# ForJadeForest/DistillCLIP

Measured on AMD Instinct MI355X. Metric: image-text pairs/sec (distill step), higher is better.
Workload: dtype bf16; 1 GPU; l_clip.yaml dual distill: ViT-B/32 CLIP teacher -> weight-shared ViT(6x768,24h,R2) + text(4x768,12h,R2) students, 224px/77tok, losses out_l1+out_cos+0.1*cos_diff, fwd+loss+bwd+AdamW; global_batch=512, batch_per_gpu=512, parallelism=dp1, gradient_exchange=none, negatives=local (reference training_step semantics), optimizer_in_step=True, teacher_residual=fp16, saved_gelu_derivative=u8 fixed point, clock_probe=True

## Files before the change

distillclip_amd/csrc/encoder.cpp:

```cpp
#include <math.h>
#include <stdlib.h>
#include <string.h>
#include <new>
#include <vector>
#include "common.h"

namespace {

#define CK(expr)                      \
    do {                              \
        int _rc = (expr);             \
        if (_rc != DCLIP_OK) return _rc; \
    } while (0)

inline size_t up256(size_t x) { return (x + 255) & ~(size_t)255; }

struct Bump {
    char* base; size_t off;
    explicit Bump(void* b) : base((char*)b), off(0) {}
    template <class T> T* take(size_t n) {
        T* p = base ? (T*)(base + off) : nullptr;
        off += up256(n * sizeof(T));
        return p;
    }
// ... 605 lines not shown
    return DCLIP_OK;
}

extern "C" int dclip_encoder_backward(const dclip_encoder* e, const void* input, const void* patches, int64_t B, const void* const* params,
                                      void* const* grads, const void* wcache, void* workspace, size_t ws_bytes, dclip_encoder_run* run,
                                      const float* d_last_representation, const float* const* d_rep, const float* d_emb,
                                      const dclip_attn_maps* maps, dclip_bucket_cb on_bucket, void* cb_user, void* st) {
    DCLIP_REQUIRE(e && (input || patches) && params && grads && wcache && workspace && run && d_last_representation, "dclip_encoder_backward: null argument");
    const Plan& p = e->p;
    const bf16_t* ext_patches = (const bf16_t*)patches;
    DCLIP_REQUIRE(!ext_patches || p.image, "dclip_encoder_backward: patches: image towers only");
    DCLIP_REQUIRE(p.train, "dclip_encoder_backward: the frozen teacher tower (kind 0) has no backward");
    ExecMaps<const float> gm;
    CK(exec_maps<const float>(p, maps, maps ? maps->d_score : nullptr, maps ? maps->d_prob : nullptr, run, "dclip_encoder_backward", gm));
    if (p.mixing && gm.prob_bits) {
        const size_t need = dclip_attn_maps_bwd_workspace_bytes(B, p.H, p.N);
        DCLIP_REQUIRE(maps->scratch && maps->scratch_bytes >= need,
                      "dclip_encoder_backward: probability-map gradients of a head-mixing tower need %zu bytes of maps scratch", need);
    }
    Work w;
    layout(p, B, true, workspace, w);
    DCLIP_REQUIRE(ws_bytes >= w.bytes, "dclip_encoder_backward: workspace too small");
    const bf16_t* W = (const bf16_t*)wcache;
    const int64_t N = p.N, D = p.D, F = p.F, E = p.E, M = B * N;
    const int nex = p.L * p.R;
    const bool pruned = (run->flags & RUN_PRUNED) != 0;
    DCLIP_REQUIRE(!pruned || !(d_rep && d_rep[nex - 1]),
                  "dclip_encoder_backward: a gradient for the hidden state of block execution %d, which the forward ran on the class / EOT "
                  "rows only (request that hidden state in the forward, or set DCLIP_PRUNE_LAST=0)", nex - 1);
    DCLIP_REQUIRE(!pruned || !(gm.score[nex - 1] || gm.prob[nex - 1]),
                  "dclip_encoder_backward: a map gradient for block execution %d, which the forward ran on the class / EOT rows only", nex - 1);
    auto GR = [&](int i) -> float* { return i < 0 ? nullptr : (float*)grads[i]; };
    hipStream_t hs = (hipStream_t)st;

    if (run->flags & RUN_SEEDS_CLEAR) run->flags &= ~RUN_SEEDS_CLEAR;
    else CK(clear_backward_seeds(p, w, M, B, pruned, st));
    CK(dclip_cast_bf16(d_last_representation, w.dout, B * E, st));
    if (p.student) {
        if (GR(p.head.head_w)) CK(dclip_gemm_tn_acc(w.dout, E, w.hf, D, GR(p.head.head_w), D, B, E, D, 1, w.tn_ws, w.tn_ws_bytes, st));
        if (GR(p.head.head_b)) CK(dclip_colsum_acc(w.dout, E, GR(p.head.head_b), B, E, st));
    } else if (GR(p.head.head_w)) {
        CK(dclip_gemm_tn_acc(w.hf, D, w.dout, E, GR(p.head.head_w), E, B, D, E, 1, w.tn_ws, w.tn_ws_bytes, st));
    }
    CK(gemm(w.dout, E, W + p.w_head_t, E, w.dh, D, B, D, E, nullptr, 0, nullptr, nullptr, nullptr, 0, DCLIP_OUT_BF16, 0, nullptr, st));
    const int R = p.R;
    bf16_t* gb_last = w.gb_f2 + (int64_t)(R - 1) * M * D;
    CK(dclip_layernorm_bwd(w.dh, D, 0, (const float*)(pruned ? w.compact.xout : w.X[nex]), D, pruned ? nullptr : w.pick, PF(params, p.head.norm_w), w.meanf,
                           w.rstdf, pruned ? w.Gc : w.G, D, gb_last, D, GR(p.head.norm_w), GR(p.head.norm_b), GR(bexec(p, (nex - 1) / p.R, 0).f2b), B, D, st));
    if (on_bucket) on_bucket(cb_user, 0);

    for (int ei = nex - 1; ei >= 0; --ei) {
        const int l = ei / p.R, r = ei % p.R;
        const auto& bw = p.bw[l];
        const ExecSave& s = w.ex[ei];
        const BX bx = bexec(p, l, r);
        const float *wl = nullptr, *ww = nullptr;
        float *gl = nullptr, *gw = nullptr;
        if (p.mixing) { wl = PF(params, bx.cl); ww = PF(params, bx.cw); gl = GR(bx.cl); gw = GR(bx.cw); }
        bf16_t* gb_f2 = w.gb_f2 + (int64_t)r * M * D;
        bf16_t* gb_pr = w.gb_pr + (int64_t)r * M * D;
        bf16_t* dbig = w.dbig + (int64_t)r * M * F;
        bf16_t* dqkv = w.dqkv + (int64_t)r * M * 3 * D;
        const int64_t MR = (int64_t)R * M;
        const ExecSave& s0 = w.ex[ei - r];
        const bool compact = pruned && ei == nex - 1;
        const RowSet rs = compact ? w.compact : full_rows(w, ei, M);
        const int64_t Mx = rs.rows;
        const int64_t MRw = pruned && l == p.L - 1 ? (int64_t)(R - 1) * M + B : MR;
        if (d_rep && d_rep[ei]) CK(dclip_axpy_f32(w.G, d_rep[ei], gb_f2, M * D, GR(bx.f2b), D, st));
        CK(dclip_gemm_nt(gb_f2, D, W + bw.fc2_t, D, dbig, F, Mx, F, D, 1.f, nullptr, DCLIP_ACT_MULAUX, rs.z, nullptr, nullptr, 0, DCLIP_OUT_BF16, 0, nullptr,
                         GR(bx.f1b), st));
        if (r == 0 && GR(bx.f2w)) CK(dclip_gemm_tn_acc(w.gb_f2, D, s0.u, F, GR(bx.f2w), F, MRw, D, F, wsplits(MRw, D, F), w.tn_ws, w.tn_ws_bytes, st));
        if (r == 0 && GR(bx.f1w)) CK(dclip_gemm_tn_acc(w.dbig, F, s0.h2, D, GR(bx.f1w), D, MRw, F, D, wsplits(MRw, F, D), w.tn_ws, w.tn_ws_bytes, st));
        CK(gemm(dbig, F, W + bw.fc1_t, F, w.dh, D, Mx, D, F, nullptr, 0, nullptr, nullptr, nullptr, 0, DCLIP_OUT_BF16, 0, nullptr, st));
        CK(dclip_layernorm_bwd(w.dh, D, 0, (const float*)rs.x_mid, D, nullptr, PF(params, bx.n2w), rs.mean2, rs.rstd2, compact ? w.Gc : w.G, D, gb_pr, D,
                               GR(bx.n2w), GR(bx.n2b), GR(bx.prb), Mx, D, st));
        if (r == 0 && GR(bx.prw)) CK(dclip_gemm_tn_acc(w.gb_pr, D, s0.ctx, D, GR(bx.prw), D, MRw, D, D, wsplits(MRw, D, D), w.tn_ws, w.tn_ws_bytes, st));
        bf16_t* dctx = w.dh;
        if (!compact) {
            CK(gemm(gb_pr, D, W + bw.proj_t, D, dctx, D, M, D, D, nullptr, 0, nullptr, nullptr, nullptr, 0, DCLIP_OUT_BF16, 0, nullptr, st));
        } else {
            bf16_t* dctx_c = dqkv;
            CK(gemm(gb_pr, D, W + bw.proj_t, D, dctx_c, D, B, D, D, nullptr, 0, nullptr, nullptr, nullptr, 0, DCLIP_OUT_BF16, 0, nullptr, st));
            CK(dclip_rows_expand(dctx_c, dctx, w.pick, B, N, D * 2, st));
            CK(dclip_rows_expand(w.Gc, w.G, w.pick, B, N, D * 4, st));
        }
        const MapGrad mg{gm.score[ei], gm.prob[ei], maps ? maps->scratch : nullptr, maps ? maps->scratch_bytes : 0};
        CK(attn_backward(w.path, p, s, w, wl, ww, gl, gw, dctx, dqkv, B, mg.d_score || mg.d_prob ? &mg : nullptr,
                         compact && (run->flags & RUN_PRUNED_ATTN) ? w.pick : nullptr, st));
        if (r == 0 && GR(bx.qkvw)) CK(dclip_gemm_tn_acc(w.dqkv, 3 * D, s0.h1, D, GR(bx.qkvw), D, MR, 3 * D, D, wsplits(MR, 3 * D, D), w.tn_ws, w.tn_ws_bytes, st));
        if (r == 0 && params[bx.qkvb] && GR(bx.qkvb)) CK(dclip_colsum_acc(w.dqkv, 3 * D, GR(bx.qkvb), MR, 3 * D, st));
        CK(gemm(dqkv, 3 * D, W + bw.qkv_t, 3 * D, w.dh, D, M, D, 3 * D, nullptr, 0, nullptr, nullptr, nullptr, 0, DCLIP_OUT_BF16, 0, nullptr, st));
        bf16_t* gb_next = ei > 0 ? w.gb_f2 + (int64_t)((ei - 1) % R) * M * D : w.Gb;
        CK(dclip_layernorm_bwd(w.dh, D, 0, (const float*)w.X[ei], D, nullptr, PF(params, bx.n1w), s.mean1, s.rstd1, w.G, D, gb_next, D, GR(bx.n1w), GR(bx.n1b),
                               ei > 0 ? GR(bexec(p, (ei - 1) / p.R, 0).f2b) : nullptr, M, D, st));
        if (r == 0 && on_bucket) on_bucket(cb_user, 1 + (p.L - 1 - l));
    }

    const Plan::EmbP& em = p.emb;
    const bool pre_ln = em.ln_w >= 0;
    if (d_emb && !pre_ln) CK(dclip_axpy_f32(w.G, d_emb, w.Gb, M * D, nullptr, D, st));
    if (hipMemsetAsync(w.tok_sum, 0, (size_t)N * D * 4, hs) != hipSuccess) { dclip_set_error("dclip_encoder_backward: memset failed"); return DCLIP_ELAUNCH; }
    const float* Ge = w.G;
    if (pre_ln) {
        if (hipMemsetAsync(w.G0, 0, (size_t)M * D * 4, hs) != hipSuccess) { dclip_set_error("dclip_encoder_backward: memset failed"); return DCLIP_ELAUNCH; }
        CK(dclip_layernorm_bwd(w.G, D, 1, (const float*)w.x0, D, nullptr, PF(params, em.ln_w), w.mean0, w.rstd0, w.G0, D, w.Gb, D, GR(em.ln_w), GR(em.ln_b),
                               nullptr, M, D, st));
        if (d_emb) CK(dclip_axpy_f32(w.G0, d_emb, w.Gb, M * D, nullptr, D, st));
        Ge = w.G0;
    }
    if (em.w >= 0) {
        const int64_t K = p.K;
        const bf16_t* rows = ext_patches ? ext_patches : w.patches;
        if (GR(em.w)) CK(dclip_gemm_tn_acc(w.Gb, D, rows, K, GR(em.w), K, M, D, K, wsplits(M, D, K), w.tn_ws, w.tn_ws_bytes, st));
        if (GR(em.bias) || GR(em.cls) || GR(em.pos)) {
            CK(dclip_batch_sum_acc(Ge, w.tok_sum, B, N, D, st));
            CK(dclip_token_table_bwd(w.tok_sum, GR(em.pos), GR(em.cls), GR(em.bias), N, D, p.image ? 1 : 0, st));
        }
        if (GR(em.table)) {
            CK(gemm(w.Gb, D, W + p.w_embed_t, D, w.demb, K, M, K, D, nullptr, 0, nullptr, nullptr, nullptr, 0, DCLIP_OUT_F32, 0, nullptr, st));
            CK(dclip_embed_scatter_add((const int64_t*)input, w.demb, 1, GR(em.table), M, K, p.c.vocab, st));
        }
    } else {
// ... 22 lines not shown
```

distillclip_amd/csrc/gemm.hip:

```cpp

#include "gemm_common.h"
#include <atomic>

using namespace dgemm;

namespace {

constexpr int TILE_BYTES = (BM / 16) * (BK / 32) * SUB;
constexpr int CLD = BN + 4;
constexpr int NT_LDS = (4 * TILE_BYTES > BM * CLD * 4) ? 4 * TILE_BYTES : BM * CLD * 4;


__device__ __forceinline__ void stage_operand(const bf16_t* __restrict__ G, int64_t ld, int row0, int rows_max,
                                              int k0, char* lds_tile, int wave, int lane) {
    const int L = lane * 16;
    const int X = swz(L);
    const int r = X >> 6, c = (X >> 4) & 3;
#pragma unroll
    for (int s = 0; s < 4; ++s) {
        const int sub = wave * 4 + s;
        const int rb = sub >> 1, kb = sub & 1;
        int row = row0 + rb * 16 + r;
        row = row < rows_max ? row : rows_max - 1;
        const bf16_t* src = G + (int64_t)row * ld + (k0 + kb * 32 + c * 8);
// ... 614 lines not shown
    float* cs = (float*)smem;
#pragma unroll
    for (int i = 0; i < 4; ++i)
#pragma unroll
        for (int j = 0; j < 4; ++j)
#pragma unroll
            for (int r = 0; r < 4; ++r)
                cs[(wp * 64 + i * 16 + (lane >> 4) * 4 + r) * TCLD + wq * 64 + j * 16 + (lane & 15)] = acc[i][j][r];
    __syncthreads();
#pragma unroll 4
    for (int it = 0; it < 64; ++it) {
        const int rl = wave * 32 + (it >> 1), cl = (it & 1) * 64 + lane;
        const int row = p0 + rl, col = q0 + cl;
        if (row < p.P && col < p.Q) unsafeAtomicAdd(p.out + (int64_t)row * p.ldo + col, cs[rl * TCLD + cl]);
    }
}

__device__ __forceinline__ void tn_half_sources(const bf16_t* __restrict__ G, int64_t ld, int m0, int c0, int wave, int lane,
                                                const char* (&src)[2]) {
#pragma unroll
    for (int s = 0; s < 2; ++s) {
        const int piece = wave * 2 + s;
        const int r = piece * 4 + (lane >> 4);
        const int lc = (lane & 15) ^ tn_key(r);
        src[s] = (const char*)(G + (int64_t)(m0 + r) * ld + c0 + lc * 8);
    }
}
__device__ __forceinline__ void stage_half_tn(const char* const (&src)[2], int64_t chunk_off, char* buf, int wave) {
#pragma unroll
    for (int s = 0; s < 2; ++s)
        __builtin_amdgcn_global_load_lds((gbl_void*)(src[s] + chunk_off), (lds_void*)(buf + (wave * 2 + s) * 1024), 16, 0, 0);
}

__global__ __launch_bounds__(512) void gemm_tn256_kernel(GemmTN p) {
    extern __shared__ __attribute__((aligned(16))) char smem[];
    const int tid = threadIdx.x, lane = tid & 63;
    const int wave = __builtin_amdgcn_readfirstlane(tid >> 6);
    const int wr = wave >> 2, wc = wave & 3;

    const int tiles = p.tiles_p * p.tiles_q;
    const int t = xcd_remap(blockIdx.x, tiles * p.splits);
    const int split = t / tiles, tile = t - split * tiles;
    const int tq = tile % p.tiles_q, tp = tile / p.tiles_q;
    const int p0 = tp * 256, q0 = tq * 256;
    const int m_begin = split * p.chunk;
    const int m_end = min(p.M, m_begin + p.chunk);
    if (m_begin >= m_end) return;
    const int nk = (m_end - m_begin) / TC;
    const int nload = 4 * nk;

    f32x4 acc[8][4];
#pragma unroll
    for (int i = 0; i < 8; ++i)
#pragma unroll
        for (int j = 0; j < 4; ++j) acc[i][j] = f32x4{0.f, 0.f, 0.f, 0.f};

    const char* srcs[4][2];
    tn_half_sources(p.B, p.ldb, m_begin, q0, wave, lane, srcs[0]);
    tn_half_sources(p.B, p.ldb, m_begin, q0 + 128, wave, lane, srcs[1]);
    tn_half_sources(p.A, p.lda, m_begin, p0, wave, lane, srcs[2]);
    tn_half_sources(p.A, p.lda, m_begin, p0 + 128, wave, lane, srcs[3]);
    const int64_t step_b = (int64_t)TC * p.ldb * 2, step_a = (int64_t)TC * p.lda * 2;
    auto issue = [&](int l) {
        const int kt = l >> 2, w = l & 3;
        char* buf = smem + ((kt & 1) * 4 + w) * HT;
        if (w == 0) stage_half_tn(srcs[0], kt * step_b, buf, wave);
        else if (w == 1) stage_half_tn(srcs[1], kt * step_b, buf, wave);
        else if (w == 2) stage_half_tn(srcs[2], kt * step_a, buf, wave);
        else stage_half_tn(srcs[3], kt * step_a, buf, wave);
    };
    auto stamp = [&](int k) {
        if (p.stamps && tid == 0) {
            if (k == 3) WAIT_VMCNT(0);
            p.stamps[6 * (int64_t)blockIdx.x + k] = __builtin_readcyclecounter();
            if (k == 0) p.stamps[6 * (int64_t)blockIdx.x + 4] = __builtin_amdgcn_s_memrealtime();
            if (k == 3) p.stamps[6 * (int64_t)blockIdx.x + 5] = __builtin_amdgcn_s_memrealtime();
        }
    };
    stamp(0);
    const int npro = nload < 6 ? nload : 6;
#pragma unroll
    for (int l = 0; l < 6; ++l)
        if (l < npro) issue(l);
    if (nload > 4) WAIT_VMCNT(4); else WAIT_VMCNT(0);
    __builtin_amdgcn_s_barrier();
    stamp(1);
    if (wr == 1) __builtin_amdgcn_s_barrier();

    const int a_off = (2 + wr) * HT;
    const int b_off = (wc >> 1) * HT;
    const int bcol = (wc & 1) * 64;
    bf16x8 af[4][2], b0[2][2], b1[2][2];

    for (int kt = 0; kt < nk; ++kt) {
        const char* base = smem + (kt & 1) * 4 * HT;
        const char* at = base + a_off;
        const char* bt = base + b_off;
        const int k4 = kt * 4;
#pragma unroll
        for (int j = 0; j < 2; ++j) {
            const unsigned a0 = tr_frag_base(bt, bcol + j * 16, lane), a1 = tr_frag_base(bt, bcol + (2 + j) * 16, lane);
            b0[j][0] = tr_frag_asm<0>(a0); b0[j][1] = tr_frag_asm<32 * 256>(a0);
            b1[j][0] = tr_frag_asm<0>(a1); b1[j][1] = tr_frag_asm<32 * 256>(a1);
        }
        __builtin_amdgcn_sched_barrier(0);
#pragma unroll
        for (int i = 0; i < 4; ++i) {
            const unsigned a0 = tr_frag_base(at, i * 16, lane);
            af[i][0] = tr_frag_asm<0>(a0); af[i][1] = tr_frag_asm<32 * 256>(a0);
// ... 29 lines not shown
        __builtin_amdgcn_sched_barrier(0);
        __builtin_amdgcn_s_barrier();
        __builtin_amdgcn_s_setprio(1);
#pragma unroll
        for (int kb = 0; kb < 2; ++kb)
#pragma unroll
            for (int i = 0; i < 4; ++i) {
#pragma unroll
                for (int j = 0; j < 2; ++j)
                    acc[4 + i][j] = __builtin_amdgcn_mfma_f32_16x16x32_bf16(af[i][kb], b0[j][kb], acc[4 + i][j], 0, 0, 0);
#pragma unroll
                for (int j = 0; j < 2; ++j)
                    acc[4 + i][2 + j] = __builtin_amdgcn_mfma_f32_16x16x32_bf16(af[i][kb], b1[j][kb], acc[4 + i][2 + j], 0, 0, 0);
            }
        __builtin_amdgcn_s_setprio(0);
        __builtin_amdgcn_s_barrier();
    }
    if (wr == 0) __builtin_amdgcn_s_barrier();
    stamp(2);

    float* cs = (float*)smem;
    constexpr int CL = 256 + 4;
#pragma unroll
    for (int q = 0; q < 4; ++q) {
        __syncthreads();
#pragma unroll
        for (int i = 0; i < 2; ++i)
#pragma unroll
            for (int j = 0; j < 4; ++j)
#pragma unroll
                for (int r = 0; r < 4; ++r)
                    cs[(wr * 32 + i * 16 + (lane >> 4) * 4 + r) * CL + wc * 64 + j * 16 + (lane & 15)] = acc[q * 2 + i][j][r];
        __syncthreads();
        if (p.partial) {
            float* dst = p.partial + ((int64_t)split * tiles + tile) * 65536;
#pragma unroll 4
            for (int it = 0; it < 8; ++it) {
                const int sl = (tid >> 6) + it * 8;
                const int rt = (sl >> 5) * 128 + q * 32 + (sl & 31);
                *(float4*)(dst + rt * 256 + (tid & 63) * 4) = *(const float4*)&cs[sl * CL + (tid & 63) * 4];
            }
        } else {
#pragma unroll 4
            for (int it = 0; it < 32; ++it) {
                const int sl = (tid >> 8) + it * 2;
                const int row = p0 + (sl >> 5) * 128 + q * 32 + (sl & 31);
                const int col = q0 + (tid & 255);
                unsafeAtomicAdd(p.out + (int64_t)row * p.ldo + col, cs[sl * CL + (tid & 255)]);
            }
        }
    }
    stamp(3);
}

__global__ __launch_bounds__(256) void tn256_reduce_kernel(const float* __restrict__ partial, int splits, int tiles, int tiles_q,
                                                           float* __restrict__ out, int64_t ldo) {
    const int idx = blockIdx.x * 256 + threadIdx.x;
    const int tile = idx >> 14, rt = (idx >> 6) & 255, c4 = idx & 63;
    if (tile >= tiles) return;
    const float* src = partial + (int64_t)tile * 65536 + rt * 256 + c4 * 4;
    float4 a = *(const float4*)src;
    for (int s = 1; s < splits; ++s) {
        const float4 v = *(const float4*)(src + (int64_t)s * tiles * 65536);
        a.x += v.x; a.y += v.y; a.z += v.z; a.w += v.w;
    }
    float* o = out + (int64_t)((tile / tiles_q) * 256 + rt) * ldo + (tile % tiles_q) * 256 + c4 * 4;
    float4 cur = *(const float4*)o;
    cur.x += a.x; cur.y += a.y; cur.z += a.z; cur.w += a.w;
    *(float4*)o = cur;
}

__global__ __launch_bounds__(256) void colsum_kernel(const bf16_t* __restrict__ X, int64_t ld, float* __restrict__ db,
                                                     int M, int N, int rows_per_block) {
    const int col = blockIdx.x * 256 + threadIdx.x;
    if (col >= N) return;
    const int r0 = blockIdx.y * rows_per_block;
    const int r1 = min(M, r0 + rows_per_block);
    float s0 = 0.f, s1 = 0.f, s2 = 0.f, s3 = 0.f;
    int r = r0;
    for (; r + 3 < r1; r += 4) {
        s0 += bf2f(X[(int64_t)r * ld + col]);
        s1 += bf2f(X[(int64_t)(r + 1) * ld + col]);
        s2 += bf2f(X[(int64_t)(r + 2) * ld + col]);
        s3 += bf2f(X[(int64_t)(r + 3) * ld + col]);
    }
// ... 200 lines not shown
    chunk = ((chunk + TC - 1) / TC) * TC;
    p.chunk = chunk;
    p.splits = (int)((M + chunk - 1) / chunk);
    const int grid = p.tiles_p * p.tiles_q * p.splits;
    const bool fast = M % TC == 0 && P >= 8 && Q >= 8;
    if (fast && P % 256 == 0 && Q % 256 == 0 && (P / 256) * (Q / 256) >= 16 && M >= 4096) {
        GemmTN q = p;
        q.tiles_p = (int)(P / 256); q.tiles_q = (int)(Q / 256);
        const int tiles = q.tiles_p * q.tiles_q;
        int s = (256 + tiles / 2) / tiles;
        if (s < 1) s = 1;
        int ch = (int)((M + s - 1) / s);
        ch = ((ch + TC - 1) / TC) * TC;
        q.chunk = ch;
        q.splits = (int)((M + ch - 1) / ch);
        TraceScope tr2(DCLIP_TRACE_GEMM_TN, 2.0 * (double)M * (double)P * (double)Q, 2.0 * ((double)M * P + (double)M * Q) + 4.0 * (double)P * Q, stream, (int)M, (int)P, (int)Q, 256);
        static const int tn_partial = [] { const char* e = getenv("DCLIP_TN_PARTIAL"); return e ? atoi(e) : 1; }();
        const size_t need = (size_t)tiles * q.splits * 65536 * sizeof(float);
        const bool part = tn_partial != 0 && workspace && ws_bytes >= need && ldo % 4 == 0 && ((uintptr_t)dW % 16) == 0 && q.splits > 1;
        if (!part && q.splits > 1) g_tn_atomic_fallbacks.fetch_add(1, std::memory_order_relaxed);
        q.partial = part ? (float*)workspace : nullptr;
        hipLaunchKernelGGL(gemm_tn256_kernel, dim3(tiles * q.splits), dim3(512), 8 * HT, (hipStream_t)stream, q);
        if (part)
            hipLaunchKernelGGL(tn256_reduce_kernel, dim3((unsigned)(tiles * 64)), dim3(256), 0, (hipStream_t)stream, (const float*)workspace,
                               q.splits, tiles, q.tiles_q, dW, ldo);
        return dclip_check_launch("dclip_gemm_tn_acc");
    }
    TraceScope tr(DCLIP_TRACE_GEMM_TN, 2.0 * (double)M * (double)P * (double)Q, 2.0 * ((double)M * P + (double)M * Q) + 4.0 * (double)P * Q, stream, (int)M, (int)P, (int)Q, 128);
    if (fast) hipLaunchKernelGGL(gemm_tn_glds_kernel, dim3(grid), dim3(256), TN_LDS, (hipStream_t)stream, p);
    else hipLaunchKernelGGL(gemm_tn_kernel, dim3(grid), dim3(256), 4 * TTILE, (hipStream_t)stream, p);
    return dclip_check_launch("dclip_gemm_tn_acc");
}

extern "C" int dclip_colsum_acc(const void* X, int64_t ld, float* db, int64_t M, int64_t N, void* stream) {
    DCLIP_REQUIRE(X && db && M > 0 && N > 0, "dclip_colsum_acc: bad argument");
    const int colblocks = (int)((N + 255) / 256);
    int rows_per_block = (int)((M * colblocks + 511) / 512);
    rows_per_block = rows_per_block < 16 ? 16 : (rows_per_block > 512 ? 512 : (rows_per_block + 3) & ~3);
    dim3 grid((unsigned)((N + 255) / 256), (unsigned)((M + rows_per_block - 1) / rows_per_block));
    if (N % 8 == 0 && ld % 8 == 0 && ((uintptr_t)X & 15) == 0)
        hipLaunchKernelGGL(colsum8_kernel, grid, dim3(256), 0, (hipStream_t)stream, (const bf16_t*)X, ld, db, (int)M, (int)N,
                           rows_per_block);
    else
        hipLaunchKernelGGL(colsum_kernel, grid, dim3(256), 0, (hipStream_t)stream, (const bf16_t*)X, ld, db, (int)M, (int)N,
                           rows_per_block);
    return dclip_check_launch("dclip_colsum_acc");
}
```

distillclip_amd/ops.py:

```python
import torch

from ._lib import lib

ACT = {'none': 0, None: 0, 'quickgelu': 1, 'gelu': 2, 'dgelu': 3, 'mulaux': 4, 'gelu_save': 5, 'quickgelu_save': 6}
OUT_DTYPE = {torch.bfloat16: 0, torch.float32: 1, torch.float16: 2}
DG_LO, DG_STEP = -0.13, 1.26 / 255.0


def _p(t):
    return 0 if t is None else t.data_ptr()


def _stream():
    return torch.cuda.current_stream().cuda_stream


def _chk(*ts):
    for t in ts:
        if t is not None and not t.is_cuda:
            raise RuntimeError('distillclip_amd ops need CUDA(HIP) tensors; there is no CPU fallback')


def gemm_nt(a, b, *, bias=None, act=None, aux_in=None, aux_out=None, residual=None, out=None, out_dtype=torch.bfloat16,
            alpha=1.0, row_group=0, rowadd=None, out_rows=None, colsum=None):
    _chk(a, b, bias, aux_in, aux_out, residual, out, rowadd)
    assert a.dtype == torch.bfloat16 and b.dtype == torch.bfloat16 and a.dim() == 2 and b.dim() == 2
    assert a.stride(1) == 1 and b.stride(1) == 1
    M, K = a.shape
    N = b.shape[0]
    if out is None:
        rows = out_rows if out_rows is not None else M
        out = torch.empty((rows, N), dtype=out_dtype, device=a.device)
# ... 2 lines not shown
    if act in ('gelu_save', 'quickgelu_save') and aux_out is not None:
        assert aux_out.dtype == torch.uint8 and aux_out.stride(0) == out.stride(0)
    if act == 'mulaux':
        assert aux_in.dtype == torch.uint8 and aux_in.stride(0) == out.stride(0)
    if residual is not None:
        assert residual.dtype == (torch.float16 if out.dtype == torch.float16 else torch.float32)
    lib().dclip_gemm_nt(_p(a), a.stride(0), _p(b), b.stride(0), _p(out), out.stride(0), M, N, K, float(alpha),
                        _p(bias), ACT[act], _p(aux_in), _p(aux_out), _p(residual), ldr,
                        OUT_DTYPE[out.dtype], row_group, _p(rowadd), _p(colsum), _stream())
    return out


_TN_WS = {}


def _tn_workspace(device):
    key = (device, _stream())
    ws = _TN_WS.get(key)
    if ws is None:
        ws = _TN_WS[key] = torch.empty(lib().dclip_gemm_tn_workspace_bytes(), dtype=torch.uint8, device=device)
    return ws


def gemm_tn_acc(a, b, dw, splits=4, workspace=True):
    _chk(a, b, dw)
    assert a.dtype == torch.bfloat16 and b.dtype == torch.bfloat16 and dw.dtype == torch.float32
    M, P = a.shape
    Q = b.shape[1]
    assert b.shape[0] == M and tuple(dw.shape) == (P, Q) and dw.stride(1) == 1
    ws = _tn_workspace(a.device) if workspace else None
    lib().dclip_gemm_tn_acc(_p(a), a.stride(0), _p(b), b.stride(0), _p(dw), dw.stride(0), M, P, Q, splits, _p(ws),
                            0 if ws is None else ws.numel(), _stream())
    return dw


def colsum_acc(x, db):
    _chk(x, db)
    assert x.dtype == torch.bfloat16 and db.dtype == torch.float32
    lib().dclip_colsum_acc(_p(x), x.stride(0), _p(db), x.shape[0], x.shape[1], _stream())
    return db


def layernorm_fwd(x, gamma, beta, *, row_index=None, out_dtype=torch.bfloat16, eps=1e-5, save_stats=True):
    _chk(x, gamma, beta, row_index)
    assert x.dtype in (torch.float32, torch.float16) and x.dim() == 2 and x.stride(1) == 1
    M = row_index.numel() if row_index is not None else x.shape[0]
    D = x.shape[1]
    y = torch.empty((M, D), dtype=out_dtype, device=x.device)
    mean = torch.empty(M, dtype=torch.float32, device=x.device) if save_stats else None
    rstd = torch.empty(M, dtype=torch.float32, device=x.device) if save_stats else None
    fn = lib().dclip_layernorm_fwd_f16 if x.dtype == torch.float16 else lib().dclip_layernorm_fwd
    fn(_p(x), x.stride(0), _p(row_index), _p(gamma), _p(beta), _p(y), D, OUT_DTYPE[out_dtype], _p(mean), _p(rstd), M, D, eps, _stream())
    return y, mean, rstd


def layernorm_bwd(dy, x, gamma, mean, rstd, dx_acc, *, row_index=None, dx_bf16=None, dgamma=None, dbeta=None, colsum=None):
    _chk(dy, x, gamma, mean, rstd, dx_acc, dx_bf16, dgamma, dbeta)
    M, D = dy.shape
    lib().dclip_layernorm_bwd(_p(dy), dy.stride(0), 1 if dy.dtype == torch.float32 else 0, _p(x), x.stride(0),
                              _p(row_index), _p(gamma), _p(mean), _p(rstd), _p(dx_acc), dx_acc.stride(0), _p(dx_bf16),
                              dx_bf16.stride(0) if dx_bf16 is not None else 0, _p(dgamma), _p(dbeta), _p(colsum), M, D, _stream())


def attn_nt(a, lda, bm, ldb, B, H, N, hd, alpha=1.0, out_dtype=torch.float32):
    Np = (N + 7) // 8 * 8
    c = torch.empty((B, H, N, Np), dtype=out_dtype, device=a.device)
# ... 280 lines not shown
```

include/dclip.h:

```cpp
#ifndef DCLIP_H
#define DCLIP_H
#include <stddef.h>
#include <stdint.h>
#ifdef __cplusplus
extern "C" {
#endif

#define DCLIP_OK 0
#define DCLIP_EINVAL (-1)
#define DCLIP_ELAUNCH (-2)

int dclip_version(void);
int dclip_runtime_check(void);
const char* dclip_arch(void);
const char* dclip_last_error_string(void);

#define DCLIP_ACT_NONE 0
#define DCLIP_ACT_QUICKGELU 1
#define DCLIP_ACT_GELU 2
#define DCLIP_ACT_DGELU 3
#define DCLIP_ACT_MULAUX 4
#define DCLIP_ACT_GELU_SAVE 5
#define DCLIP_ACT_QUICKGELU_SAVE 6
#define DCLIP_OUT_BF16 0
#define DCLIP_OUT_F32 1
#define DCLIP_OUT_F16 2

int dclip_gemm_nt(const void* A, int64_t lda, const void* B, int64_t ldb, void* C, int64_t ldc,
                  int64_t M, int64_t N, int64_t K, float alpha, const float* bias, int act,
                  const void* aux_in, void* aux_out, const void* residual, int64_t ldr, int out_dtype,
                  int64_t row_group, const float* rowadd, float* colsum_acc, void* stream);

size_t dclip_gemm_tn_workspace_bytes(void);
int64_t dclip_gemm_tn_atomic_fallbacks(void);
int dclip_gemm_tn_acc(const void* A, int64_t lda, const void* B, int64_t ldb, float* dW, int64_t ldo,
                      int64_t M, int64_t P, int64_t Q, int splits, void* workspace, size_t ws_bytes, void* stream);

int dclip_colsum_acc(const void* X, int64_t ld, float* db, int64_t M, int64_t N, void* stream);

int dclip_layernorm_fwd(const float* x, int64_t ldx, const int32_t* row_index, const float* gamma, const float* beta,
                        void* y, int64_t ldy, int out_f32, float* mean, float* rstd, int64_t M, int64_t D, float eps,
                        void* stream);
int dclip_layernorm_fwd_f16(const void* x, int64_t ldx, const int32_t* row_index, const float* gamma, const float* beta,
                            void* y, int64_t ldy, int out_dtype, float* mean, float* rstd, int64_t M, int64_t D, float eps,
                            void* stream);
int dclip_layernorm_bwd(const void* dy, int64_t lddy, int dy_f32, const float* x, int64_t ldx, const int32_t* row_index,
                        const float* gamma, const float* mean, const float* rstd, float* dx_acc, int64_t lddx,
                        void* dx_bf16, int64_t lddb, float* dgamma, float* dbeta, float* colsum_acc, int64_t M, int64_t D,
                        void* stream);

int dclip_attn_nt(const void* A, int64_t lda, const void* Bm, int64_t ldb, void* C, int out_f32, int64_t B, int64_t H,
                  int64_t N, int64_t Np, int64_t hd, float alpha, void* stream);
int dclip_attn_nn(const void* A, const void* Bm, int64_t ldb, void* C, int64_t ldc, int64_t B, int64_t H, int64_t N,
                  int64_t Np, int64_t hd, float alpha, int a_blocked, void* stream);
int dclip_attn_tn(const void* A, const void* Bm, int64_t ldb, void* C, int64_t ldc, int64_t B, int64_t H, int64_t N,
                  int64_t Np, int64_t hd, float alpha, int a_blocked, void* stream);
int dclip_attn_fused_fwd(const void* qkv, int64_t ldq, void* ctx, int64_t ldc, int64_t B, int64_t H, int64_t N, int64_t hd,
                         float scale, int causal, void* stream);
int dclip_attn_stream_fwd(const void* qkv, int64_t ldq, void* ctx, int64_t ldc, int64_t B, int64_t H, int64_t N, int64_t hd,
                          float scale, void* stream);
int dclip_attn_softmax_fwd(const float* S, const float* Wl, const float* Ww, void* P, void* R, int64_t B, int64_t H,
                           int64_t N, int64_t Np, int causal, void* stream);
int dclip_attn_softmax_bwd(const void* dR, const void* P, const void* S, int scores_bf16, const float* Wl, const float* Ww,
                           void* dS, float* dWl, float* dWw, int64_t B, int64_t H, int64_t N, int64_t Np, void* stream);
int dclip_attn_mix_supported(int64_t H, int64_t N, int64_t hd);
size_t dclip_attn_mix_bwd_workspace_bytes(int64_t B, int64_t H, int64_t N);
void dclip_attn_mix_debug_stamps(void* fwd, void* bwd_a, void* bwd_b);
int dclip_attn_mix_fwd(const void* qkv, int64_t ld, const float* Wl, const float* Ww, void* R, float* stats, int64_t B, int64_t H,
                       int64_t N, int64_t Np, int64_t hd, float scale, void* stream);
// ... 167 lines not shown
```

Before: 18620 pairs/s.

## Group per-layer weight-gradient TN GEMMs into one persistent split-K launch

Batches the four weight-gradient TN GEMMs of each layer (fc2, fc1, qkv, proj) into a single grouped kernel. The kernel balances K-slabs of all problems across a fixed number of workgroups, writes partials to a workspace and reduces them in a follow-up kernel. It aims to cut launch count and load imbalance, and to raise CU utilisation over separate split-K launches with atomics. The cost is that all four GEMMs now wait until after attention backward, plus extra partial-buffer traffic. It is on by default, can be switched off with an env var, and falls back to separate calls if constraints fail.

```diff
diff --git a/distillclip_amd/csrc/encoder.cpp b/distillclip_amd/csrc/encoder.cpp
--- a/distillclip_amd/csrc/encoder.cpp
+++ b/distillclip_amd/csrc/encoder.cpp
@@ -661,6 +661,7 @@
                   "dclip_encoder_backward: a map gradient for block execution %d, which the forward ran on the class / EOT rows only", nex - 1);
     auto GR = [&](int i) -> float* { return i < 0 ? nullptr : (float*)grads[i]; };
     hipStream_t hs = (hipStream_t)st;
+    static const bool tn_grouped = [] { const char* e = getenv("DCLIP_TN_GROUPED"); return e ? atoi(e) != 0 : true; }();
 
     if (run->flags & RUN_SEEDS_CLEAR) run->flags &= ~RUN_SEEDS_CLEAR;
     else CK(clear_backward_seeds(p, w, M, B, pruned, st));
@@ -696,15 +697,16 @@
         const RowSet rs = compact ? w.compact : full_rows(w, ei, M);
         const int64_t Mx = rs.rows;
         const int64_t MRw = pruned && l == p.L - 1 ? (int64_t)(R - 1) * M + B : MR;
+        const bool wg_each = r == 0 && !tn_grouped;
         if (d_rep && d_rep[ei]) CK(dclip_axpy_f32(w.G, d_rep[ei], gb_f2, M * D, GR(bx.f2b), D, st));
         CK(dclip_gemm_nt(gb_f2, D, W + bw.fc2_t, D, dbig, F, Mx, F, D, 1.f, nullptr, DCLIP_ACT_MULAUX, rs.z, nullptr, nullptr, 0, DCLIP_OUT_BF16, 0, nullptr,
                          GR(bx.f1b), st));
-        if (r == 0 && GR(bx.f2w)) CK(dclip_gemm_tn_acc(w.gb_f2, D, s0.u, F, GR(bx.f2w), F, MRw, D, F, wsplits(MRw, D, F), w.tn_ws, w.tn_ws_bytes, st));
-        if (r == 0 && GR(bx.f1w)) CK(dclip_gemm_tn_acc(w.dbig, F, s0.h2, D, GR(bx.f1w), D, MRw, F, D, wsplits(MRw, F, D), w.tn_ws, w.tn_ws_bytes, st));
+        if (wg_each && GR(bx.f2w)) CK(dclip_gemm_tn_acc(w.gb_f2, D, s0.u, F, GR(bx.f2w), F, MRw, D, F, wsplits(MRw, D, F), w.tn_ws, w.tn_ws_bytes, st));
+        if (wg_each && GR(bx.f1w)) CK(dclip_gemm_tn_acc(w.dbig, F, s0.h2, D, GR(bx.f1w), D, MRw, F, D, wsplits(MRw, F, D), w.tn_ws, w.tn_ws_bytes, st));
         CK(gemm(dbig, F, W + bw.fc1_t, F, w.dh, D, Mx, D, F, nullptr, 0, nullptr, nullptr, nullptr, 0, DCLIP_OUT_BF16, 0, nullptr, st));
         CK(dclip_layernorm_bwd(w.dh, D, 0, (const float*)rs.x_mid, D, nullptr, PF(params, bx.n2w), rs.mean2, rs.rstd2, compact ? w.Gc : w.G, D, gb_pr, D,
                                GR(bx.n2w), GR(bx.n2b), GR(bx.prb), Mx, D, st));
-        if (r == 0 && GR(bx.prw)) CK(dclip_gemm_tn_acc(w.gb_pr, D, s0.ctx, D, GR(bx.prw), D, MRw, D, D, wsplits(MRw, D, D), w.tn_ws, w.tn_ws_bytes, st));
+        if (wg_each && GR(bx.prw)) CK(dclip_gemm_tn_acc(w.gb_pr, D, s0.ctx, D, GR(bx.prw), D, MRw, D, D, wsplits(MRw, D, D), w.tn_ws, w.tn_ws_bytes, st));
         bf16_t* dctx = w.dh;
         if (!compact) {
             CK(gemm(gb_pr, D, W + bw.proj_t, D, dctx, D, M, D, D, nullptr, 0, nullptr, nullptr, nullptr, 0, DCLIP_OUT_BF16, 0, nullptr, st));
@@ -717,7 +719,19 @@
         const MapGrad mg{gm.score[ei], gm.prob[ei], maps ? maps->scratch : nullptr, maps ? maps->scratch_bytes : 0};
         CK(attn_backward(w.path, p, s, w, wl, ww, gl, gw, dctx, dqkv, B, mg.d_score || mg.d_prob ? &mg : nullptr,
                          compact && (run->flags & RUN_PRUNED_ATTN) ? w.pick : nullptr, st));
-        if (r == 0 && GR(bx.qkvw)) CK(dclip_gemm_tn_acc(w.dqkv, 3 * D, s0.h1, D, GR(bx.qkvw), D, MR, 3 * D, D, wsplits(MR, 3 * D, D), w.tn_ws, w.tn_ws_bytes, st));
+        if (wg_each && GR(bx.qkvw)) CK(dclip_gemm_tn_acc(w.dqkv, 3 * D, s0.h1, D, GR(bx.qkvw), D, MR, 3 * D, D, wsplits(MR, 3 * D, D), w.tn_ws, w.tn_ws_bytes, st));
+        if (r == 0 && !wg_each) {
+            const dclip_tn_problem all[4] = {{w.gb_f2, D, s0.u, F, GR(bx.f2w), F, MRw, D, F}, {w.dbig, F, s0.h2, D, GR(bx.f1w), D, MRw, F, D},
+                                             {w.dqkv, 3 * D, s0.h1, D, GR(bx.qkvw), D, MR, 3 * D, D}, {w.gb_pr, D, s0.ctx, D, GR(bx.prw), D, MRw, D, D}};
+            dclip_tn_problem pb[4];
+            int npb = 0, grouped = 0;
+            for (const dclip_tn_problem& q : all) if (q.dW) pb[npb++] = q;
+            if (npb) CK(dclip_gemm_tn_acc_grouped(pb, npb, w.tn_ws, w.tn_ws_bytes, 0, &grouped, st));
+            if (!grouped)
+                for (int i = 0; i < npb; ++i)
+                    CK(dclip_gemm_tn_acc(pb[i].A, pb[i].lda, pb[i].B, pb[i].ldb, pb[i].dW, pb[i].ldo, pb[i].M, pb[i].P, pb[i].Q,
+                                         wsplits(pb[i].M, pb[i].P, pb[i].Q), w.tn_ws, w.tn_ws_bytes, st));
+        }
         if (r == 0 && params[bx.qkvb] && GR(bx.qkvb)) CK(dclip_colsum_acc(w.dqkv, 3 * D, GR(bx.qkvb), MR, 3 * D, st));
         CK(gemm(dqkv, 3 * D, W + bw.qkv_t, 3 * D, w.dh, D, M, D, 3 * D, nullptr, 0, nullptr, nullptr, nullptr, 0, DCLIP_OUT_BF16, 0, nullptr, st));
         bf16_t* gb_next = ei > 0 ? w.gb_f2 + (int64_t)((ei - 1) % R) * M * D : w.Gb;
diff --git a/distillclip_amd/csrc/gemm.hip b/distillclip_amd/csrc/gemm.hip
--- a/distillclip_amd/csrc/gemm.hip
+++ b/distillclip_amd/csrc/gemm.hip
@@ -670,21 +670,16 @@
         __builtin_amdgcn_global_load_lds((gbl_void*)(src[s] + chunk_off), (lds_void*)(buf + (wave * 2 + s) * 1024), 16, 0, 0);
 }
 
-__global__ __launch_bounds__(512) void gemm_tn256_kernel(GemmTN p) {
+template <bool ATOMICS>
+__device__ __forceinline__ void tn256_segment(const bf16_t* A, int64_t lda, const bf16_t* B, int64_t ldb,
+                                              int p0, int q0, int m_begin, int nk, float* partial, int slot, float* out,
+                                              int64_t ldo, unsigned long long* stamps) {
     extern __shared__ __attribute__((aligned(16))) char smem[];
-    const int tid = threadIdx.x, lane = tid & 63;
+    int tid_ = threadIdx.x;
+    asm volatile("" : "+v"(tid_));
+    const int tid = tid_, lane = tid & 63;
     const int wave = __builtin_amdgcn_readfirstlane(tid >> 6);
     const int wr = wave >> 2, wc = wave & 3;
-
-    const int tiles = p.tiles_p * p.tiles_q;
-    const int t = xcd_remap(blockIdx.x, tiles * p.splits);
-    const int split = t / tiles, tile = t - split * tiles;
-    const int tq = tile % p.tiles_q, tp = tile / p.tiles_q;
-    const int p0 = tp * 256, q0 = tq * 256;
-    const int m_begin = split * p.chunk;
-    const int m_end = min(p.M, m_begin + p.chunk);
-    if (m_begin >= m_end) return;
-    const int nk = (m_end - m_begin) / TC;
     const int nload = 4 * nk;
 
     f32x4 acc[8][4];
@@ -694,11 +689,11 @@
         for (int j = 0; j < 4; ++j) acc[i][j] = f32x4{0.f, 0.f, 0.f, 0.f};
 
     const char* srcs[4][2];
-    tn_half_sources(p.B, p.ldb, m_begin, q0, wave, lane, srcs[0]);
-    tn_half_sources(p.B, p.ldb, m_begin, q0 + 128, wave, lane, srcs[1]);
-    tn_half_sources(p.A, p.lda, m_begin, p0, wave, lane, srcs[2]);
-    tn_half_sources(p.A, p.lda, m_begin, p0 + 128, wave, lane, srcs[3]);
-    const int64_t step_b = (int64_t)TC * p.ldb * 2, step_a = (int64_t)TC * p.lda * 2;
+    tn_half_sources(B, ldb, m_begin, q0, wave, lane, srcs[0]);
+    tn_half_sources(B, ldb, m_begin, q0 + 128, wave, lane, srcs[1]);
+    tn_half_sources(A, lda, m_begin, p0, wave, lane, srcs[2]);
+    tn_half_sources(A, lda, m_begin, p0 + 128, wave, lane, srcs[3]);
+    const int64_t step_b = (int64_t)TC * ldb * 2, step_a = (int64_t)TC * lda * 2;
     auto issue = [&](int l) {
         const int kt = l >> 2, w = l & 3;
         char* buf = smem + ((kt & 1) * 4 + w) * HT;
@@ -708,11 +703,11 @@
         else stage_half_tn(srcs[3], kt * step_a, buf, wave);
     };
     auto stamp = [&](int k) {
-        if (p.stamps && tid == 0) {
+        if (stamps && tid == 0) {
             if (k == 3) WAIT_VMCNT(0);
-            p.stamps[6 * (int64_t)blockIdx.x + k] = __builtin_readcyclecounter();
-            if (k == 0) p.stamps[6 * (int64_t)blockIdx.x + 4] = __builtin_amdgcn_s_memrealtime();
-            if (k == 3) p.stamps[6 * (int64_t)blockIdx.x + 5] = __builtin_amdgcn_s_memrealtime();
+            stamps[6 * (int64_t)blockIdx.x + k] = __builtin_readcyclecounter();
+            if (k == 0) stamps[6 * (int64_t)blockIdx.x + 4] = __builtin_amdgcn_s_memrealtime();
+            if (k == 3) stamps[6 * (int64_t)blockIdx.x + 5] = __builtin_amdgcn_s_memrealtime();
         }
     };
     stamp(0);
@@ -808,8 +803,8 @@
                 for (int r = 0; r < 4; ++r)
                     cs[(wr * 32 + i * 16 + (lane >> 4) * 4 + r) * CL + wc * 64 + j * 16 + (lane & 15)] = acc[q * 2 + i][j][r];
         __syncthreads();
-        if (p.partial) {
-            float* dst = p.partial + ((int64_t)split * tiles + tile) * 65536;
+        if (!ATOMICS || partial) {
+            float* dst = partial + (int64_t)slot * 65536;
 #pragma unroll 4
             for (int it = 0; it < 8; ++it) {
                 const int sl = (tid >> 6) + it * 8;
@@ -822,11 +817,121 @@
                 const int sl = (tid >> 8) + it * 2;
                 const int row = p0 + (sl >> 5) * 128 + q * 32 + (sl & 31);
                 const int col = q0 + (tid & 255);
-                unsafeAtomicAdd(p.out + (int64_t)row * p.ldo + col, cs[sl * CL + (tid & 255)]);
+                unsafeAtomicAdd(out + (int64_t)row * ldo + col, cs[sl * CL + (tid & 255)]);
             }
         }
     }
     stamp(3);
+}
+
+__global__ __launch_bounds__(512) void gemm_tn256_kernel(GemmTN p) {
+    const int tiles = p.tiles_p * p.tiles_q;
+    const int t = xcd_remap(blockIdx.x, tiles * p.splits);
+    const int split = t / tiles, tile = t - split * tiles;
+    const int tq = tile % p.tiles_q, tp = tile / p.tiles_q;
+    const int m_begin = split * p.chunk;
+    const int m_end = min(p.M, m_begin + p.chunk);
+    if (m_begin >= m_end) return;
+    tn256_segment<true>(p.A, p.lda, p.B, p.ldb, tp * 256, tq * 256, m_begin, (m_end - m_begin) / TC,
+                        p.partial, split * tiles + tile, p.out, p.ldo, p.stamps);
+}
+
+struct TnGroupProb {
+    const bf16_t* A; const bf16_t* B; float* out;
+    int64_t lda, ldb, ldo;
+    int tiles_q, tiles;
+    int nk;
+    int full, rem;
+    int wg0;
+    int tile0, slab0;
+    int rpos0, rtile0;
+};
+struct TnGroup {
+    TnGroupProb pr[4];
+    int n, S;
+    int F, Gr, Rt;
+    int G, tiles;
+    float* partial;
+};
+__host__ __device__ __forceinline__ int tn_rcut(const TnGroup& g, int j) { return (int)((unsigned)j * (unsigned)g.Rt / (unsigned)g.Gr); }
+__host__ __device__ __forceinline__ int tn_rcuts_le(const TnGroup& g, int x) {
+    if (g.Gr <= 1) return 0;
+    const int c = (int)((((unsigned)x + 1u) * (unsigned)g.Gr - 1u) / (unsigned)g.Rt);
+    return c < g.Gr - 1 ? c : g.Gr - 1;
+}
+__host__ __device__ __forceinline__ int tn_tile_slot(const TnGroup& g, const TnGroupProb& q, int tl, int& count) {
+    int base = q.slab0 + tl * q.full, cnt = q.full;
+    if (q.rem > 0) {
+        const int r0 = q.rpos0 + tl * q.rem;
+        const int c0 = tn_rcuts_le(g, r0);
+        base += q.rtile0 + tl + c0;
+        cnt += 1 + tn_rcuts_le(g, r0 + q.rem - 1) - c0;
+    } else base += q.rtile0 + tn_rcuts_le(g, q.rpos0);
+    count = cnt;
+    return base;
+}
+
+__global__ __launch_bounds__(512) void gemm_tn256_grouped_kernel(TnGroup g) {
+    const int w = xcd_remap(blockIdx.x, g.G);
+    const int before = (int)((unsigned)w * (unsigned)g.F / (unsigned)g.G);
+    const bool slab_wg = (int)((unsigned)(w + 1) * (unsigned)g.F / (unsigned)g.G) > before;
+    int x = 0, xe = 1;
+    if (!slab_wg) {
+        const int j = w - before;
+        if (j >= g.Gr) return;
+        x = tn_rcut(g, j);
+        xe = tn_rcut(g, j + 1);
+    }
+    while (x < xe) {
+        const int key = slab_wg ? before : x;
+        int pi = 0;
+        for (int i = 1; i < g.n; ++i) if (key >= (slab_wg ? g.pr[i].wg0 : g.pr[i].rpos0)) pi = i;
+        const TnGroupProb& q = g.pr[__builtin_amdgcn_readfirstlane(pi)];
+        int tl, c0, len, slot, adv;
+        if (slab_wg) {
+            const int local = before - q.wg0;
+            const int slab = local / q.tiles;
+            int cnt;
+            tl = local - slab * q.tiles;
+            c0 = slab * g.S; len = g.S; adv = 1;
+            slot = tn_tile_slot(g, q, tl, cnt) + slab;
+        } else {
+            const int rel = x - q.rpos0;
+            tl = rel / q.rem;
+            const int off = rel - tl * q.rem;
+            c0 = q.full * g.S + off; len = min(q.rem - off, xe - x); adv = len;
+            slot = q.slab0 + (tl + 1) * q.full + q.rtile0 + tl + tn_rcuts_le(g, x);
+        }
+        tl = __builtin_amdgcn_readfirstlane(tl); c0 = __builtin_amdgcn_readfirstlane(c0);
+        len = __builtin_amdgcn_readfirstlane(len); slot = __builtin_amdgcn_readfirstlane(slot);
+        const int tp = tl / q.tiles_q, tq = tl - tp * q.tiles_q;
+        tn256_segment<false>(q.A, q.lda, q.B, q.ldb, tp * 256, tq * 256, c0 * TC, len, g.partial, slot, nullptr, 0, nullptr);
+        x += adv;
+        WAIT_VMCNT(0);
+        __syncthreads();
+    }
+}
+
+__global__ __launch_bounds__(256) void tn256_group_reduce_kernel(TnGroup g) {
+    const int tile = blockIdx.x >> 6;
+    int pi = 0;
+    for (int i = 1; i < g.n; ++i) if (tile >= g.pr[i].tile0) pi = i;
+    const TnGroupProb& q = g.pr[pi];
+    const int tl = tile - q.tile0;
+    int cnt;
+    const int slot = tn_tile_slot(g, q, tl, cnt);
+    const int idx = (blockIdx.x & 63) * 256 + threadIdx.x;
+    const int rt = idx >> 6, c4 = idx & 63;
+    const float* src = g.partial + (int64_t)slot * 65536 + rt * 256 + c4 * 4;
+    float4 a = *(const float4*)src;
+    for (int s = 1; s < cnt; ++s) {
+        const float4 v = *(const float4*)(src + (int64_t)s * 65536);
+        a.x += v.x; a.y += v.y; a.z += v.z; a.w += v.w;
+    }
+    float* o = q.out + (int64_t)((tl / q.tiles_q) * 256 + rt) * q.ldo + (tl % q.tiles_q) * 256 + c4 * 4;
+    float4 cur = *(const float4*)o;
+    cur.x += a.x; cur.y += a.y; cur.z += a.z; cur.w += a.w;
+    *(float4*)o = cur;
 }
 
 __global__ __launch_bounds__(256) void tn256_reduce_kernel(const float* __restrict__ partial, int splits, int tiles, int tiles_q,
@@ -1093,6 +1198,72 @@
     return dclip_check_launch("dclip_gemm_tn_acc");
 }
 
+namespace {
+bool tn_group_plan(TnGroup& g, int G) {
+    int64_t T = 0;
+    int nk_max = 0;
+    for (int i = 0; i < g.n; ++i) { T += (int64_t)g.pr[i].tiles * g.pr[i].nk; nk_max = g.pr[i].nk > nk_max ? g.pr[i].nk : nk_max; }
+    if (T * G >= (1LL << 31)) return false;
+    int S = (int)((T + G - 1) / G);
+    for (;; ++S) {
+        int64_t F = 0;
+        for (int i = 0; i < g.n; ++i) F += (int64_t)g.pr[i].tiles * (g.pr[i].nk / S);
+        const int64_t rest = T - F * S;
+        if (rest == 0 || (G > F && (rest + (G - F) - 1) / (G - F) <= S) || S > nk_max) {
+            g.S = S; g.F = (int)F; g.Rt = (int)rest; g.Gr = (int)(rest < G - F ? rest : G - F); g.G = G;
+            break;
+        }
+    }
+    int wg = 0, tile = 0, slab = 0, rpos = 0, rtile = 0;
+    for (int i = 0; i < g.n; ++i) {
+        TnGroupProb& q = g.pr[i];
+        q.full = q.nk / g.S; q.rem = q.nk - q.full * g.S;
+        q.wg0 = wg; q.tile0 = tile; q.slab0 = slab; q.rpos0 = rpos; q.rtile0 = rtile;
+        wg += q.tiles * q.full; tile += q.tiles; slab += q.tiles * q.full;
+        if (q.rem > 0) { rpos += q.tiles * q.rem; rtile += q.tiles; }
+    }
+    g.tiles = tile;
+    return true;
+}
+}
+
+extern "C" int dclip_gemm_tn_acc_grouped(const dclip_tn_problem* problems, int n, void* workspace, size_t ws_bytes, int wgs, int* grouped,
+                                         void* stream) {
+    DCLIP_REQUIRE(problems && grouped, "dclip_gemm_tn_acc_grouped: null argument");
+    DCLIP_REQUIRE(n >= 1 && n <= DCLIP_TN_GROUP_MAX, "dclip_gemm_tn_acc_grouped: n=%d problems, must be 1..%d", n, DCLIP_TN_GROUP_MAX);
+    DCLIP_REQUIRE(wgs >= 0 && wgs <= 4096, "dclip_gemm_tn_acc_grouped: wgs=%d, must be 0 (one per CU) .. 4096", wgs);
+    *grouped = 0;
+    TnGroup g;
+    double flops = 0.0, bytes = 0.0;
+    int64_t m_max = 0;
+    for (int i = 0; i < n; ++i) {
+        const dclip_tn_problem& s = problems[i];
+        DCLIP_REQUIRE(s.A && s.B && s.dW, "dclip_gemm_tn_acc_grouped: null operand in problem %d", i);
+        DCLIP_REQUIRE(s.M > 0 && s.P > 0 && s.Q > 0, "dclip_gemm_tn_acc_grouped: empty problem %d", i);
+        if (s.P % 256 || s.Q % 256 || s.M % TC || s.M >= (1LL << 31) || s.P >= (1 << 20) || s.Q >= (1 << 20) || s.lda % 8 || s.ldb % 8 || s.ldo % 4 ||
+            ((uintptr_t)s.A % 16) || ((uintptr_t)s.B % 16) || ((uintptr_t)s.dW % 16) || s.lda < s.P || s.ldb < s.Q || s.ldo < s.Q)
+            return DCLIP_OK;
+        TnGroupProb& q = g.pr[i];
+        q.A = (const bf16_t*)s.A; q.B = (const bf16_t*)s.B; q.out = s.dW; q.lda = s.lda; q.ldb = s.ldb; q.ldo = s.ldo;
+        q.tiles_q = (int)(s.Q / 256); q.tiles = (int)(s.P / 256) * q.tiles_q; q.nk = (int)(s.M / TC);
+        flops += 2.0 * (double)s.M * (double)s.P * (double)s.Q;
+        bytes += 2.0 * ((double)s.M * s.P + (double)s.M * s.Q) + 4.0 * (double)s.P * s.Q;
+        m_max = s.M > m_max ? s.M : m_max;
+    }
+    for (int i = n; i < DCLIP_TN_GROUP_MAX; ++i) g.pr[i] = TnGroupProb{};
+    g.n = n;
+    g.partial = (float*)workspace;
+    if (!tn_group_plan(g, wgs > 0 ? wgs : 256)) return DCLIP_OK;
+    int cnt;
+    const int slots = tn_tile_slot(g, g.pr[n - 1], g.pr[n - 1].tiles - 1, cnt) + cnt;
+    if (!workspace || ((uintptr_t)workspace % 16) || ws_bytes < (size_t)slots * 65536 * sizeof(float)) return DCLIP_OK;
+    TraceScope tr(DCLIP_TRACE_GEMM_TN, flops, bytes, stream, (int)m_max, g.tiles, n, 256);
+    hipLaunchKernelGGL(gemm_tn256_grouped_kernel, dim3((unsigned)g.G), dim3(512), 8 * HT, (hipStream_t)stream, g);
+    hipLaunchKernelGGL(tn256_group_reduce_kernel, dim3((unsigned)(g.tiles * 64)), dim3(256), 0, (hipStream_t)stream, g);
+    *grouped = 1;
+    return dclip_check_launch("dclip_gemm_tn_acc_grouped");
+}
+
 extern "C" int dclip_colsum_acc(const void* X, int64_t ld, float* db, int64_t M, int64_t N, void* stream) {
     DCLIP_REQUIRE(X && db && M > 0 && N > 0, "dclip_colsum_acc: bad argument");
     const int colblocks = (int)((N + 255) / 256);
diff --git a/distillclip_amd/ops.py b/distillclip_amd/ops.py
--- a/distillclip_amd/ops.py
+++ b/distillclip_amd/ops.py
@@ -1,3 +1,5 @@
+import ctypes
+
 import torch
 
 from ._lib import lib
@@ -66,6 +68,26 @@
     lib().dclip_gemm_tn_acc(_p(a), a.stride(0), _p(b), b.stride(0), _p(dw), dw.stride(0), M, P, Q, splits, _p(ws),
                             0 if ws is None else ws.numel(), _stream())
     return dw
+
+
+class _TnProblem(ctypes.Structure):
+    _fields_ = [('A', ctypes.c_void_p), ('lda', ctypes.c_int64), ('B', ctypes.c_void_p), ('ldb', ctypes.c_int64),
+                ('dW', ctypes.c_void_p), ('ldo', ctypes.c_int64), ('M', ctypes.c_int64), ('P', ctypes.c_int64), ('Q', ctypes.c_int64)]
+
+
+def gemm_tn_acc_grouped(problems, wgs=0, workspace=None):
+    pb = (_TnProblem * len(problems))()
+    for q, (a, b, dw) in zip(pb, problems):
+        _chk(a, b, dw)
+        assert a.dtype == torch.bfloat16 and b.dtype == torch.bfloat16 and dw.dtype == torch.float32
+        assert a.shape[0] == b.shape[0] and tuple(dw.shape) == (a.shape[1], b.shape[1])
+        assert a.stride(1) == 1 and b.stride(1) == 1 and dw.stride(1) == 1
+        q.A, q.lda, q.B, q.ldb, q.dW, q.ldo = _p(a), a.stride(0), _p(b), b.stride(0), _p(dw), dw.stride(0)
+        q.M, q.P, q.Q = a.shape[0], a.shape[1], b.shape[1]
+    ws = _tn_workspace(problems[0][0].device) if workspace is None else workspace
+    grouped = ctypes.c_int(0)
+    lib().dclip_gemm_tn_acc_grouped(pb, len(problems), _p(ws), ws.numel(), wgs, ctypes.byref(grouped), _stream())
+    return bool(grouped.value)
 
 
 def colsum_acc(x, db):
diff --git a/include/dclip.h b/include/dclip.h
--- a/include/dclip.h
+++ b/include/dclip.h
@@ -35,6 +35,16 @@
 int64_t dclip_gemm_tn_atomic_fallbacks(void);
 int dclip_gemm_tn_acc(const void* A, int64_t lda, const void* B, int64_t ldb, float* dW, int64_t ldo,
                       int64_t M, int64_t P, int64_t Q, int splits, void* workspace, size_t ws_bytes, void* stream);
+
+#define DCLIP_TN_GROUP_MAX 4
+typedef struct dclip_tn_problem {
+    const void* A; int64_t lda;
+    const void* B; int64_t ldb;
+    float* dW; int64_t ldo;
+    int64_t M, P, Q;
+} dclip_tn_problem;
+int dclip_gemm_tn_acc_grouped(const dclip_tn_problem* problems, int n, void* workspace, size_t ws_bytes, int wgs, int* grouped,
+                              void* stream);
 
 int dclip_colsum_acc(const void* X, int64_t ld, float* db, int64_t M, int64_t N, void* stream);
 
```

New measurement: 18720 pairs/s (median of 6 runs). About the same (+0.6%).
